# alberto-paparella/MusicRecommendation

Measured on AMD Instinct MI355X. Metric: scored (test-user,song) pairs/sec, ItemBasedModel, 1/2/4/8 MI355X + mAP@10, higher is better.
Workload: dtype int64

## Files before the change

include/mr_engine.h:

```cpp
#ifndef MR_ENGINE_H
#define MR_ENGINE_H

#include <stdint.h>
#include <stddef.h>

#ifdef __cplusplus
extern "C" {
#endif

#define MR_OK          0
#define MR_E_INVALID  -1
#define MR_E_HIP      -2
#define MR_E_OOM      -3
#define MR_E_STATE    -4
#define MR_E_IO       -5
#define MR_E_PARSE    -6
#define MR_E_RCCL     -7

#define MR_UBM 0
#define MR_IBM 1

#define MR_OUT_F32 0
#define MR_OUT_F64 1

// ... 35 lines not shown

int mr_create(const mr_options* opt, mr_ctx** out);
int mr_destroy(mr_ctx* ctx);

int mr_load(mr_ctx* ctx, const mr_dataset* d);

int mr_shard_info(const mr_ctx* ctx, int32_t* song_lo, int32_t* song_hi, int32_t* n_test_users);

int mr_launch_info(const mr_ctx* ctx, int32_t* shape, int32_t* block_songs, int32_t* n_tiles);

int mr_batch_info(const mr_ctx* ctx, int32_t* batch, int32_t* chunk, int32_t* n_chunks);

int mr_route_info(const mr_ctx* ctx, int32_t* route, int32_t* n_rows, int64_t* pool_entries);

int mr_topk_mode(const mr_ctx* ctx, int32_t* candidate_only);

int mr_cooc_stats(mr_ctx* ctx, int64_t* index_nnz, int64_t* consumed, int64_t* build_reads);

typedef struct mr_cooc_bytes_t {
  int64_t heavy_rows, light_rows;
  int64_t heavy_reads, light_reads;
  int64_t heavy_index_bytes, light_index_bytes;
  int64_t heavy_visits;
  int64_t consumed_bytes;
  int64_t group_tiles;
  int64_t n_groups;
  int64_t index_sparse_entries, index_dense_songs;
  int64_t consumed_sparse_entries, consumed_dense_songs;
} mr_cooc_bytes_t;
int mr_cooc_bytes(mr_ctx* ctx, mr_cooc_bytes_t* out);
// ... 174 lines not shown
```

musicrecommendation_amd/_lib.py:

```python
from __future__ import annotations

import ctypes
import os
from ctypes import POINTER, c_char_p, c_double, c_int, c_int32, c_int64, c_void_p

_HERE = os.path.dirname(os.path.abspath(__file__))
_VARIANT = os.environ.get("MR_ENGINE_LIB", "")
LIB_PATH = os.path.join(_HERE, f"libmr_engine_{_VARIANT}.so" if _VARIANT else "libmr_engine.so")

MR_OK = 0
MR_E_INVALID = -1
MR_E_HIP = -2
MR_E_OOM = -3
MR_E_STATE = -4
MR_E_IO = -5
MR_E_PARSE = -6
MR_E_RCCL = -7
MR_TRANSPORT_AUTO, MR_TRANSPORT_COPY, MR_TRANSPORT_RCCL = 0, 1, 2
MR_UBM = 0
MR_IBM = 1
STAGE1 = {"auto": 0, "fused": 1, "separate": 2, "wide": 4}
SHAPES = {0: "separate", 1: "fused", 3: "wide"}
MR_OUT_F32 = 0
MR_OUT_F64 = 1
# ... 88 lines not shown
    def __init__(self, code: int, where: str, msg: str):
        super().__init__(f"{where}: {_ERRNAMES.get(code, code)}: {msg}")
        self.code = code


SIGNATURES = {
    "mr_options_default": (c_int, [POINTER(MrOptions)]),
    "mr_create": (c_int, [POINTER(MrOptions), POINTER(c_void_p)]),
    "mr_destroy": (c_int, [c_void_p]),
    "mr_load": (c_int, [c_void_p, POINTER(MrDataset)]),
    "mr_shard_info": (c_int, [c_void_p, POINTER(c_int32), POINTER(c_int32), POINTER(c_int32)]),
    "mr_launch_info": (c_int, [c_void_p, POINTER(c_int32), POINTER(c_int32), POINTER(c_int32)]),
    "mr_batch_info": (c_int, [c_void_p, POINTER(c_int32), POINTER(c_int32), POINTER(c_int32)]),
    "mr_route_info": (c_int, [c_void_p, POINTER(c_int32), POINTER(c_int32), POINTER(c_int64)]),
    "mr_topk_mode": (c_int, [c_void_p, POINTER(c_int32)]),
    "mr_cooc_stats": (c_int, [c_void_p, POINTER(c_int64), POINTER(c_int64), POINTER(c_int64)]),
    "mr_cooc_bytes": (c_int, [c_void_p, POINTER(MrCoocBytes)]),
    "mr_shard_tile_songs": (c_int, [POINTER(MrOptions), c_int32, c_int32, POINTER(c_int32)]),
    "mr_shard_tile_songs_n": (c_int, [POINTER(MrOptions), c_int32, c_int32, c_int32, c_int32, POINTER(c_int32)]),
    "mr_run": (c_int, [c_void_p, c_int]),
    "mr_sync": (c_int, [c_void_p]),
    "mr_graph_capture": (c_int, [c_void_p, c_int, c_int32]),
    "mr_graph_launch": (c_int, [c_void_p]),
    "mr_device_outputs": (c_int, [c_void_p, POINTER(c_void_p), POINTER(c_void_p), POINTER(c_void_p), POINTER(c_void_p)]),
    "mr_score_dense": (c_int, [c_void_p, c_int, c_void_p]),
    "mr_topk": (c_int, [c_void_p, c_int, c_int, c_void_p, c_void_p, c_void_p]),
    "mr_copy_dense": (c_int, [c_void_p, c_void_p]),
    "mr_copy_topk": (c_int, [c_void_p, c_void_p, c_void_p, c_void_p]),
    "mr_copy_topk_device": (c_int, [c_void_p, c_void_p, c_void_p]),
    "mr_copy_topk_device_async": (c_int, [c_void_p, c_void_p, c_void_p]),
# ... 112 lines not shown
```

musicrecommendation_amd/csrc/mr_engine.hip:

```cpp
#include <hip/hip_runtime.h>

#include <algorithm>
#include <atomic>
#include <climits>
#include <cmath>
#include <cstdarg>
#include <cstdio>
#include <cstdlib>
#include <cstring>
#include <limits>
#include <mutex>
#include <string>
#include <vector>

#ifndef MR_TILE_ROWS
#define MR_TILE_ROWS 32
#endif

#include "mr_engine.h"
#include "mr_internal.h"
#include "mr_par.h"


namespace {
// ... 1 lines not shown
constexpr int kThreads = 256;
constexpr int kWaves = kThreads / 64;
constexpr int kMaxTopK = 64;
constexpr int kMaxBlockSongs = 16384;
constexpr int kLdsBytes = 160 * 1024;
constexpr int kMaxWideBlockSongs = 65536;
constexpr int kMaxLdsTrainUsers = 16384;
constexpr int kStage1Chunk = 4096;
constexpr int kMaxChunks = 2048;
constexpr int kMaxFusedTrainUsers = 4096;
constexpr long long kKeyNone = -1;
constexpr int kMaxTopkTile = 1024;
constexpr int kMaxTopkLarge = 16;
constexpr int kFusedPre = 4;
constexpr int kWideMapDefault = 1;

thread_local std::string g_err = "no error";

int fail(int code, const char* fmt, ...) {
  char buf[1024];
  va_list ap;
  va_start(ap, fmt);
  vsnprintf(buf, sizeof buf, fmt, ap);
  va_end(ap);
  g_err = buf;
  return code;
}

}

// ... 73 lines not shown
#ifdef MR_STAMPS
  if (sb && threadIdx.x == 0) sb[i] = (long long)__builtin_amdgcn_s_memrealtime();
#endif
}
__device__ __forceinline__ void stamp_rt_wave(long long* sb, int i) {
#ifdef MR_STAMPS
  if (sb && (threadIdx.x & 63) == 0) sb[i] = (long long)__builtin_amdgcn_s_memrealtime();
#endif
}
__device__ __forceinline__ void stamp_val(long long* sb, int i, long long v, bool wave = false) {
#ifdef MR_STAMPS
  if (sb && (wave ? (threadIdx.x & 63) == 0 : threadIdx.x == 0)) sb[i] = v;
#endif
}
#ifdef MR_STAMPS
#define MR_STAMP(i) stamp_at(p.stamps ? p.stamps + ((size_t)blockIdx.y * gridDim.x + blockIdx.x) * kStampSlots : nullptr, (i))
#else
#define MR_STAMP(i) do {} while (0)
#endif

__device__ __forceinline__ int wave_incl_scan(int x) {
#ifndef MR_NO_DPP
  x += __builtin_amdgcn_update_dpp(0, x, 0x111, 0xf, 0xf, false);
  x += __builtin_amdgcn_update_dpp(0, x, 0x112, 0xf, 0xf, false);
  x += __builtin_amdgcn_update_dpp(0, x, 0x114, 0xf, 0xf, false);
  x += __builtin_amdgcn_update_dpp(0, x, 0x118, 0xf, 0xf, false);
  x += __builtin_amdgcn_update_dpp(0, x, 0x142, 0xa, 0xf, false);
  x += __builtin_amdgcn_update_dpp(0, x, 0x143, 0xc, 0xf, false);
#else
  const int lane = threadIdx.x & 63;
#pragma unroll
// ... 776 lines not shown
  unsigned* counter;
  long long* top_key;
  int* top_song;
  double* top_score;
  long long* stamps;
  int topk_lists;
  int n_rows, nseg;
  const int* te_row;
  const long long* seg_off;
  const int* seg_len;
  const unsigned* pool;
  unsigned long long* mm_key;
  int mm_n;
  int cand;
  const float* rsq_c;
};

template <int MODEL, typename OutT, bool FUSED>
__global__ __launch_bounds__(kThreads) void k_score(ScoreParams p) {
  extern __shared__ __align__(16) unsigned char smem_raw[];
  const int bs = p.block_songs;
  const ScoreLds L = score_lds(bs, FUSED ? p.n_tr : 0, p.topk, p.n_tiles, FUSED ? 0 : p.n_chunks);
  unsigned long long* acc = reinterpret_cast<unsigned long long*>(smem_raw + L.acc);
  unsigned* heard = reinterpret_cast<unsigned*>(smem_raw + L.heard);
  long long* wk = reinterpret_cast<long long*>(smem_raw + L.wk);
  int* ws = reinterpret_cast<int*>(smem_raw + L.ws);
  long long* fk = reinterpret_cast<long long*>(smem_raw + L.fk);
  int* fs = reinterpret_cast<int*>(smem_raw + L.fs);
  int* flag = reinterpret_cast<int*>(smem_raw + L.flag);

  int tile = blockIdx.x;
// ... 703 lines not shown
    const int e = __builtin_ctz(sm);
    sm &= sm - 1u;
    const int i = tid + e * NT;
    double score = (double)(long long)acc[i] * inv_f;
    if (MODEL == MR_IBM) score = score / p.sqrt_c[blo + i];
    const int pos = atomicAdd(counter, 1);
    if (pos < cap) { ck[pos] = __double_as_longlong(score); cs[pos] = blo + i; }
  }
  __syncthreads();
  stamp_at(sb, 11);
  const int nc = *counter;
  if (nc > cap) return false;
  rank_survivors<NT>(nc, k, ck, cs, crank, fk, fs);
  return true;
}
constexpr int kCandE = 20;

template <int MODEL, typename OutT, int NT, int KS, bool COOC>
__global__ __launch_bounds__(NT) void k_score_wide(ScoreParams p) {
  constexpr int NW = NT / 64;
  extern __shared__ __align__(16) unsigned char smem_raw[];
  const int bs = p.block_songs;
  const WideLds<NT> L = wide_lds<NT>(bs, p.topk, p.n_chunks);
  unsigned long long* acc = reinterpret_cast<unsigned long long*>(smem_raw + L.acc);
  unsigned* heard = reinterpret_cast<unsigned*>(smem_raw + L.heard);
  int* cpre = reinterpret_cast<int*>(smem_raw + L.cpre);
  int* s_scan = reinterpret_cast<int*>(smem_raw + L.s_scan);

  const int lin = blockIdx.y * gridDim.x + blockIdx.x;
  const int slot = lin >> 3;
  int bu, tile;
  if (p.xcd_remap == 2) {
    const int per_xcd = (gridDim.x * gridDim.y) >> 3;
    const int pidx = (lin & 7) * per_xcd + slot;
    tile = pidx / gridDim.y;
    bu = pidx - tile * gridDim.y;
  } else if (p.xcd_remap == 3) {
    tile = lin / gridDim.y;
    bu = lin - tile * gridDim.y;
  } else {
    bu = (slot / p.n_tiles) * 8 + (lin & 7);
    tile = slot % p.n_tiles;
  }
  if (bu >= p.n_users) return;
  const int u = p.user0 + bu;
  const int tid = threadIdx.x, lane = tid & 63, w = tid >> 6;
  const int blo = p.song_lo + tile * bs;
  const int bhi = min(p.song_hi, blo + bs);
  const int bw = bhi - blo;
  MR_STAMP(0);

  constexpr bool kPF = COOC && MR_COOC_PF > 0;
  constexpr int PF = kPF ? MR_COOC_PF : 1;
  double scp[PF];
  if constexpr (kPF) {
#pragma unroll
    for (int e = 0; e < PF; ++e) {
      const int i = tid + e * NT;
      scp[e] = i < bw ? p.sqrt_c[blo + i] : 1.0;
    }
  }
  constexpr bool kDPF = COOC && MR_COOC_DPF;
  int pf_r = -1, pf_s = 0, pf_sl = 0;
  long long pf_off = 0;
  unsigned long long pf_q = 0ull;
// ... 280 lines not shown
      for (int r = 0; r < R; ++r) {
        const int k = k0 + r * NT;
        v[r] = -1;
        q[r] = 0ull;
        if (k < cnt) {
          while (cur + 1 < nch && cpre[cur + 1] <= k) ++cur;
          const size_t idx = (size_t)cur * p.chunk + (k - cpre[cur]);
          v[r] = nv[idx];
          q[r] = (unsigned long long)nq[idx];
        }
      }
    };
    walk_tile_lists<NT, R, kSeg, unsigned long long>(tid, cnt, load_list, p.toff + (size_t)tile * p.n_tr, p.tsongs,
                                                     [&](unsigned x, unsigned long long q) { atomicAdd(&acc[x], q); });
  }
  __syncthreads();
  MR_STAMP(2);

  long long* wk = reinterpret_cast<long long*>(smem_raw + L.wk);
  int* ws = reinterpret_cast<int*>(smem_raw + L.ws);
  long long* fk = reinterpret_cast<long long*>(smem_raw + L.fk);
  int* fs = reinterpret_cast<int*>(smem_raw + L.fs);
  const int k = KS == 10 ? 10 : p.topk;
  bool have = false;
#ifdef MR_STAMPS
  long long* sbp = p.stamps ? p.stamps + ((size_t)blockIdx.y * gridDim.x + blockIdx.x) * kStampSlots : nullptr;
#else
  long long* sbp = nullptr;
#endif
  if (p.cand) {
    have = wide_cand_topk<MODEL, NT, kCandE>(p, acc, heard, blo, bw, k, smem_raw + L.gm, wk, ws,
                                             min(256, NW * k), fk, fs, sbp, have_rv, pre_rv);
    MR_STAMP(6);
  }
  if (!have) {
  const double inv_f = ldexp(1.0, -p.frac_bits);
  OutT* out = reinterpret_cast<OutT*>(p.dense_out) + (size_t)u * p.width + (blo - p.song_lo);
  long long mk = kKeyNone;
  int ms = INT_MAX;
  OutT lmn = (OutT)INFINITY, lmx = (OutT)-INFINITY;
  auto store = [&](int i, bool h, double score) {
    const OutT o = h ? (OutT)NAN : (OutT)score;
    out[i] = o;
    if (!h) {
      lmn = o < lmn ? o : lmn;
      lmx = o > lmx ? o : lmx;
    }
  };
  constexpr int EB = MR_WIDE_EB;
// ... 1109 lines not shown
    }
    __syncthreads();
    if ((tid >> 6) == 0) wave_merge_lists(nl + off, k, mk, ms, fk, fs);
    __syncthreads();
    done += nl;
    off = 1;
  }
  const size_t o = (size_t)bu * k;
  for (int r = tid; r < k; r += kThreads) {
    p.out_keys[o + r] = fk[r];
    p.out_songs[o + r] = fs[r];
    if (p.out_scores) p.out_scores[o + r] = fk[r] >= 0 ? __longlong_as_double(fk[r]) : (double)NAN;
  }
}

__global__ __launch_bounds__(256) void k_sbound(const long long* trs_off, const int* trs_users, int n_s, int nc1,
                                                int chunk, int* sbound) {
  const size_t total = (size_t)n_s * nc1;
  for (size_t i = (size_t)blockIdx.x * 256 + threadIdx.x; i < total; i += (size_t)gridDim.x * 256) {
    const int s = (int)(i / nc1);
    const long long bound = (long long)(int)(i - (size_t)s * nc1) * chunk;
    long long a = trs_off[s], b = trs_off[s + 1];
    while (a < b) {
      const long long m = (a + b) >> 1;
      if (trs_users[m] < bound) a = m + 1; else b = m;
    }
    sbound[i] = (int)a;
  }
}

// ... 85 lines not shown
  NbrKernel nbr_kernel[2] = {nullptr, nullptr};
  DevBuf<long long> tr_off, te_off, trs_off, q_song, cand_key, top_key, nbr_q;
  DevBuf<int> te_songs, trs_users, toff, nbr_v, nbr_cnt, cand_song, top_song;
  DevBuf<unsigned short> tsongs;
  DevBuf<unsigned> tpack;
  DevBuf<int2> te_rng;
  DevBuf<long long> te_q;
  DevBuf<uint2> te_sched;
  DevBuf<long long> sched_off;
  DevBuf<int> sbound;
  DevBuf<unsigned> counter;
  DevBuf<double> sqrt_c, sqrt_tr, sqrt_te, top_score;
  DevBuf<float> rsq_c;
  std::vector<int32_t> song_count;
  bool cand_on = false;
  DevBuf<unsigned char> dense;
  DevBuf<long long> stamps;
  hipEvent_t stage_ev[2] = {nullptr, nullptr};
  static constexpr int kRing = 1024;
  std::vector<hipEvent_t> ring;
  int ring_used = 0;
  bool ring_has_stage1[kRing] = {};
  long long launches[3] = {0, 0, 0};
  double ms[3] = {0, 0, 0};
  hipEvent_t win[2] = {nullptr, nullptr};
  bool win_open = false;
  bool win_stopped = false;
  void* dense_override = nullptr;
  DevBuf<unsigned long long> mm_key;
  bool mm_on = false, mm_valid = false;
// ... 19 lines not shown
  DevBuf<int4> rdesc;
  DevBuf<long long> sr_off;
  DevBuf<unsigned> sr_songs;
  DevBuf<unsigned> urec;
  DevBuf<unsigned> lrec;
  DevBuf<uint2> llrec;

  void release_data() {
    tr_off.release(); te_off.release(); trs_off.release(); q_song.release();
    cand_key.release(); top_key.release(); nbr_q.release();
    tsongs.release(); tpack.release(); te_rng.release(); te_q.release(); te_sched.release(); sched_off.release(); te_songs.release(); trs_users.release(); toff.release(); sbound.release();
    nbr_v.release(); nbr_cnt.release(); cand_song.release(); top_song.release();
    counter.release();
    sqrt_c.release(); sqrt_tr.release(); sqrt_te.release(); top_score.release();
    rsq_c.release(); cand_on = false;
    song_count = std::vector<int32_t>();
    dense.release();
    mm_key.release(); mm_on = mm_valid = false;
    stamps.release();
    flag.release();
    row_song.release(); te_row.release(); seg_len.release(); row_base.release(); seg_off.release();
    pool.release();
    rows_order.release(); row_slots.release(); sr_off.release(); sr_songs.release(); row_nnz.release();
    urec.release(); lrec.release(); llrec.release(); rdesc.release();
    cooc = CoocPlan{};
    cooc_kernel = nullptr;
    if (graph_exec) (void)hipGraphExecDestroy(graph_exec);
    if (graph) (void)hipGraphDestroy(graph);
    graph_exec = nullptr;
    graph = nullptr;
// ... 175 lines not shown
    if constexpr (MODEL == MR_IBM) {
      if (c->cooc.route == 2 && c->cooc.cooc_nt == 512) {
        if (c->opt.topk == 10)
          c->cooc_kernel = f64 ? k_score_wide<MR_IBM, double, 512, 10, true> : k_score_wide<MR_IBM, float, 512, 10, true>;
        else
          c->cooc_kernel = f64 ? k_score_wide<MR_IBM, double, 512, kMaxTopkLarge, true>
                               : k_score_wide<MR_IBM, float, 512, kMaxTopkLarge, true>;
      } else if (c->cooc.route == 2) {
        if (c->opt.topk == 10)
          c->cooc_kernel = f64 ? k_score_wide<MR_IBM, double, kWideThreads, 10, true>
                               : k_score_wide<MR_IBM, float, kWideThreads, 10, true>;
        else
          c->cooc_kernel = f64 ? k_score_wide<MR_IBM, double, kWideThreads, kMaxTopkLarge, true>
                               : k_score_wide<MR_IBM, float, kWideThreads, kMaxTopkLarge, true>;
      }
    }
  }
  c->nbr_kernel[MODEL] = k_neighbours<MODEL>;
}

int pick_shape(const mr_options& o, int n_tr, int n_te) {
  const int k = o.topk;
  if (o.stage1 == 1) return kShapeFused;
  if (o.stage1 == 2) return kShapeSeparate;
  if (o.stage1 == 4) return kShapeWide;
  if (n_tr > kMaxFusedTrainUsers && k <= kMaxTopkLarge) return kShapeWide;
  if ((long long)n_te * n_tr >= kWideMinUserPairs && k <= kMaxTopkLarge) return kShapeWide;
  return n_tr <= kMaxFusedTrainUsers ? kShapeFused : kShapeSeparate;
}

// ... 629 lines not shown
  int rc;
  if (k > 0) {
    const int cand_users = !lp.wide() ? n_te : route == 2 ? std::max(lp.batch, std::min(n_te, 65528)) : lp.batch;
    const size_t nc = (size_t)cand_users * lp.n_tiles * k;
    if ((rc = dev_alloc(c->cand_key, nc))) return rc;
    if ((rc = dev_alloc(c->cand_song, nc))) return rc;
    const size_t nk = (size_t)n_te * k;
    if ((rc = dev_alloc(c->top_key, (size_t)topk_record_bytes(nk) / 8))) return rc;
    c->top_song.p = reinterpret_cast<int*>(c->top_key.p + nk);
    c->top_song.n = nk;
    c->top_song.own = false;
    if ((rc = dev_alloc(c->top_score, (size_t)n_te * k))) return rc;
    const size_t n_ctr = lp.wide() ? (size_t)n_te : (size_t)n_te * kCounterStride;
    if ((rc = dev_alloc(c->counter, n_ctr))) return rc;
    MR_HIP(hipMemsetAsync(c->counter.p, 0, n_ctr * sizeof(unsigned), st));
  }
  const size_t esz = c->opt.out_dtype == MR_OUT_F64 ? 8 : 4;
  if ((rc = dev_alloc(c->dense, c->opt.dense ? (size_t)n_te * lp.width * esz : 1))) return rc;
  if ((rc = dev_alloc(c->flag, 1))) return rc;
  return MR_OK;
}

int setup_kernels(mr_ctx* c, const LaunchPlan& lp, int n_tr) {
  const CoocPlan& p = c->cooc;
  const int bs = lp.block_songs, k = lp.k, n_chunks = lp.n_chunks;
  const bool fused = lp.fused(), wide = lp.wide();
  {
    const char* e = std::getenv("MR_WIDE_CAND");
    const int nt = p.route == 2 ? p.cooc_nt : kWideThreads;
    c->cand_on = wide && !c->opt.dense && k >= 1 && k <= nt / 16 && !c->opt.topk_lists && bs <= kCandE * nt &&
// ... 1 lines not shown
  }
  c->wide_lds = wide ? (size_t)wide_lds<kWideThreads>(bs, k, n_chunks).total : 0;
  pick_kernels<MR_UBM>(c);
  pick_kernels<MR_IBM>(c);
  c->score_lds = wide ? c->wide_lds
                      : (size_t)score_lds(bs, fused ? n_tr : 0, k, lp.n_tiles, fused ? 0 : n_chunks).total;
  if (c->score_lds > 160 * 1024)
    return fail(MR_E_INVALID, "scoring kernel needs %zu B of LDS (> 160 KiB): lower block_songs or topk",
                c->score_lds);
  c->nbr_lds = (size_t)align16(lp.chunk * 8) + kThreads * 16 + (kThreads + 4 + kWaves) * 4;
  for (int m = 0; m < 2; ++m) {
    MR_HIP(hipFuncSetAttribute((const void*)c->score_kernel[m], hipFuncAttributeMaxDynamicSharedMemorySize,
                               (int)c->score_lds));
    MR_HIP(hipFuncSetAttribute((const void*)c->nbr_kernel[m], hipFuncAttributeMaxDynamicSharedMemorySize,
                               (int)c->nbr_lds));
  }
  if (p.route == 2) {
    const WideLds<kWideThreads> WL = p.cooc_nt == 512 ? wide_lds<512>(bs, k, n_chunks).as_wide()
                                                      : wide_lds<kWideThreads>(bs, k, n_chunks);
    c->cooc_score_lds = (size_t)WL.total;
    c->nseg = std::min(std::min(p.cooc_nt, (WL.total - WL.wk - 8) / 40), 255);
    if (c->nseg < 16) return fail(MR_E_INVALID, "co-listening route: no LDS for row descriptors");
    c->cooc_lds = (size_t)cooc_build_lds<false>(bs);
    if (p.grp > 0)
      MR_HIP(hipFuncSetAttribute(p.group_nt == 512 ? (const void*)k_cooc_group<512> : (const void*)k_cooc_group<1024>,
                                 hipFuncAttributeMaxDynamicSharedMemorySize, cooc_group_lds(bs, p.grp)));
    for (int t = 0; t < kLightTiers; ++t)
      if (int rc2 = light_tier_call(t, nullptr, 0, nullptr, CoocParams{})) return rc2;
    MR_HIP(hipFuncSetAttribute((const void*)c->cooc_kernel, hipFuncAttributeMaxDynamicSharedMemorySize,
                               (int)c->cooc_score_lds));
    MR_HIP(hipFuncSetAttribute((const void*)k_cooc_build<MR_COOC_NT, false>, hipFuncAttributeMaxDynamicSharedMemorySize,
                               (int)c->cooc_lds));
    MR_HIP(hipFuncSetAttribute((const void*)k_cooc_build<MR_COOC_NT16, true>, hipFuncAttributeMaxDynamicSharedMemorySize,
                               cooc_build_lds<true>(bs)));
  }
  if (wide && k > 0) {
    c->merge_lds = (size_t)merge_lds_bytes(k);
    MR_HIP(hipFuncSetAttribute((const void*)k_topk_merge, hipFuncAttributeMaxDynamicSharedMemorySize,
                               (int)c->merge_lds));
  }
  return MR_OK;
}

}
// ... 174 lines not shown
  if (!c) return fail(MR_E_INVALID, "null context");
  if (!c->loaded) return fail(MR_E_STATE, "mr_route_info before mr_load");
  if (route) *route = c->cooc.route;
  if (n_rows) *n_rows = c->cooc.n_rows();
  if (pool_entries) *pool_entries = c->cooc.pool_cap;
  return MR_OK;
}

int mr_topk_mode(const mr_ctx* c, int32_t* candidate_only) {
  if (!c || !candidate_only) return fail(MR_E_INVALID, "null argument");
  if (!c->loaded) return fail(MR_E_STATE, "mr_topk_mode before mr_load");
  *candidate_only = c->cand_on ? 1 : 0;
  return MR_OK;
}

int mr_cooc_stats(mr_ctx* c, int64_t* index_nnz, int64_t* consumed, int64_t* build_reads) {
  if (!c) return fail(MR_E_INVALID, "null context");
  if (!c->loaded || c->cooc.route != 2) return fail(MR_E_STATE, "mr_cooc_stats needs a context on ibm_route 2");
  if (!c->cooc_ran) return fail(MR_E_STATE, "mr_cooc_stats before an ibm run");
  MR_HIP(hipSetDevice(c->opt.device));
  std::vector<unsigned> nnz((size_t)std::max(1, c->cooc.n_rows()), 0u);
  if (c->cooc.n_rows() > 0)
    MR_HIP(hipMemcpyAsync(nnz.data(), c->row_nnz.p, (size_t)c->cooc.n_rows() * 4, hipMemcpyDeviceToHost, c->stream));
  MR_HIP(hipStreamSynchronize(c->stream));
  int64_t tot = 0, use = 0;
  for (int r = 0; r < c->cooc.n_rows(); ++r) {
    tot += nnz[r];
    use += (int64_t)nnz[r] * c->cooc.row_users[r];
  }
  if (index_nnz) *index_nnz = tot;
// ... 102 lines not shown

}

namespace {

int flush_timing(mr_ctx* c) {
  if (c->ring_used == 0) return MR_OK;
  MR_HIP(hipEventSynchronize(c->ring[(size_t)(c->ring_used - 1) * 3 + 2]));
  for (int i = 0; i < c->ring_used; ++i) {
    hipEvent_t* e = &c->ring[(size_t)i * 3];
    float t;
    if (c->ring_has_stage1[i]) { MR_HIP(hipEventElapsedTime(&t, e[0], e[1])); c->ms[0] += t; c->launches[0]++; }
    MR_HIP(hipEventElapsedTime(&t, e[1], e[2])); c->ms[1] += t; c->launches[1]++;
  }
  c->ring_used = 0;
  return MR_OK;
}

int run_cooc(mr_ctx* c) {
  hipStream_t st = c->stream;
  const CoocPlan& p = c->cooc;
  const bool timed = c->opt.time_kernels != 0;
  const int k = c->opt.topk;
  hipEvent_t* ev = nullptr;
  if (timed) {
    if (c->ring_used == mr_ctx::kRing) {
      int rc = flush_timing(c);
      if (rc) return rc;
    }
    ev = &c->ring[(size_t)c->ring_used * 3];
// ... 59 lines not shown
      lp.rows = c->rows_order.p + lr;
      lp.rdesc = c->rdesc.p + lr;
      lp.llrec = reinterpret_cast<const unsigned*>(c->llrec.p);
      lp.lstamps = c->stamps.p ? c->stamps.p + c->lstamp_off + (size_t)(lr - p.n_heavy()) * 8 : nullptr;
      hipStream_t ls = side ? c->side[t < 2 ? 0 : 1] : st;
      if (int rc2 = light_tier_call(t, ls, p.n_light_tier[t], &lp, lp)) return rc2;
      lr += p.n_light_tier[t];
    }
    if (side)
      for (int i = 0; i < 2; ++i) {
        MR_HIP(hipEventRecord(c->side_join[i], c->side[i]));
        MR_HIP(hipStreamWaitEvent(st, c->side_join[i], 0));
      }
  }
  if (timed) MR_HIP(hipEventRecord(ev[1], st));
  const int rows = mr_internal::launch_rows(65528);
  for (int y0 = 0; y0 < c->n_te; y0 += rows) {
    const int ny = std::min(rows, c->n_te - y0);
    const int remap = wide_map_opt();
    ScoreParams sp{};
    sp.chunk = c->chunk; sp.n_chunks = c->n_chunks;
    sp.n_users = ny; sp.xcd_remap = remap;
    sp.merge_rows = merge_rows_opt();
    sp.n_tr = c->n_tr;
    sp.user0 = y0;
    sp.song_lo = c->song_lo; sp.song_hi = c->song_hi; sp.width = c->width;
    sp.block_songs = c->block_songs; sp.n_tiles = c->n_tiles;
    sp.frac_bits = c->opt.frac_bits; sp.topk = k; sp.dense = c->opt.dense;
    sp.te_off = c->te_off.p; sp.te_songs = c->te_songs.p;
    sp.sqrt_c = c->sqrt_c.p; sp.q_song = c->q_song.p;
    sp.n_rows = p.n_rows(); sp.nseg = c->nseg;
    sp.te_row = c->te_row.p; sp.seg_off = c->seg_off.p; sp.seg_len = c->seg_len.p; sp.pool = c->pool.p;
    sp.dense_out = c->dense_override ? c->dense_override : (void*)c->dense.p;
    sp.cand_key = c->cand_key.p; sp.cand_song = c->cand_song.p; sp.counter = c->counter.p;
    sp.top_key = c->top_key.p; sp.top_song = c->top_song.p; sp.top_score = c->top_score.p;
    sp.stamps = y0 == 0 ? c->stamps.p : nullptr;
    sp.topk_lists = c->opt.topk_lists;
    if (c->mm_on) { sp.mm_key = c->mm_key.p; sp.mm_n = c->n_te; }
    sp.cand = c->cand_on && !sp.mm_key; sp.rsq_c = c->rsq_c.p;
    hipLaunchKernelGGL(c->cooc_kernel, dim3(c->n_tiles, (ny + 7) / 8 * 8), dim3(p.cooc_nt), c->cooc_score_lds, st, sp);
    MR_HIP(hipGetLastError());
    if (k > 0 && c->n_tiles > 1) {
      MergeParams mp{c->n_tiles, k, k, (long long)c->n_tiles * k, (long long)k, (long long)k, c->cand_key.p,
                     c->cand_song.p, c->top_key.p + (size_t)y0 * k, c->top_song.p + (size_t)y0 * k,
                     c->top_score.p + (size_t)y0 * k};
      hipLaunchKernelGGL(k_topk_merge, dim3(ny), dim3(kThreads), c->merge_lds, st, mp);
      MR_HIP(hipGetLastError());
    }
    if (c->win_open) c->win_launches++;
  }
  if (timed) MR_HIP(hipEventRecord(ev[2], st));
  return MR_OK;
}

int ensure_nbr(mr_ctx* c) {
  if (c->shape == kShapeFused || (c->nbr_v.p && c->nbr_q.p && c->nbr_cnt.p)) return MR_OK;
// ... 1 lines not shown
  if ((rc = dev_alloc(c->nbr_v, (size_t)c->batch * c->cap))) return rc;
  if ((rc = dev_alloc(c->nbr_q, (size_t)c->batch * c->cap))) return rc;
  if ((rc = dev_alloc(c->nbr_cnt, (size_t)c->batch * c->n_chunks))) return rc;
  return MR_OK;
}

int run_model(mr_ctx* c, int model) {
  if (model == MR_IBM && c->cooc.route == 2) {
    c->cooc_ran = true;
    return run_cooc(c);
  }
  hipStream_t st = c->stream;
  const bool timed = c->opt.time_kernels != 0;
  const int k = c->opt.topk;
  const int rows1 = mr_internal::launch_rows(65535), rows = mr_internal::launch_rows(65528);
  for (int user0 = 0; user0 < c->n_te; user0 += c->batch) {
    const int nb = std::min(c->batch, c->n_te - user0);
    hipEvent_t* ev = nullptr;
    if (timed) {
      if (c->ring_used == mr_ctx::kRing) {
        int rc = flush_timing(c);
        if (rc) return rc;
      }
      ev = &c->ring[(size_t)c->ring_used * 3];
      c->ring_has_stage1[c->ring_used] = c->shape != kShapeFused;
      c->ring_used++;
      MR_HIP(hipEventRecord(ev[0], st));
    }
    if (c->shape == kShapeSeparate || c->shape == kShapeWide) {
      if (!c->nbr_v.p || !c->nbr_q.p || !c->nbr_cnt.p) {
// ... 37 lines not shown
      sp.te_rng = nullptr;
#endif
      sp.trs_off = c->trs_off.p; sp.trs_users = c->trs_users.p; sp.q_song = c->q_song.p;
      sp.sqrt_tr = c->sqrt_tr.p; sp.sqrt_te = c->sqrt_te.p;
      sp.cap = c->cap;
      sp.nbr_v = c->fused ? nullptr : c->nbr_v.p + (size_t)y0 * c->cap;
      sp.nbr_q = c->fused ? nullptr : c->nbr_q.p + (size_t)y0 * c->cap;
      sp.nbr_cnt = c->fused ? nullptr : c->nbr_cnt.p + (size_t)y0 * c->n_chunks;
      sp.dense_out = c->dense_override ? c->dense_override : (void*)c->dense.p;
      sp.cand_key = c->cand_key.p; sp.cand_song = c->cand_song.p; sp.counter = c->counter.p;
      sp.top_key = c->top_key.p; sp.top_song = c->top_song.p; sp.top_score = c->top_score.p;
      sp.stamps = c->stamps.p ? c->stamps.p + (size_t)y0 * c->n_tiles * kStampSlots : nullptr;
      sp.topk_lists = c->opt.topk_lists;
      if (c->mm_on && wide) { sp.mm_key = c->mm_key.p; sp.mm_n = c->n_te; }
      sp.cand = wide && c->cand_on && !sp.mm_key; sp.rsq_c = c->rsq_c.p;
      hipLaunchKernelGGL(c->score_kernel[model], dim3(c->n_tiles, gy), dim3(wide ? kWideThreads : kThreads),
                         c->score_lds, st, sp);
      MR_HIP(hipGetLastError());
      if (wide && k > 0 && c->n_tiles > 1) {
        MergeParams mp{c->n_tiles, k, k, (long long)c->n_tiles * k, (long long)k, (long long)k, c->cand_key.p, c->cand_song.p,
                       c->top_key.p + (size_t)(user0 + y0) * k, c->top_song.p + (size_t)(user0 + y0) * k,
                       c->top_score.p + (size_t)(user0 + y0) * k};
        hipLaunchKernelGGL(k_topk_merge, dim3(ny), dim3(kThreads), c->merge_lds, st, mp);
        MR_HIP(hipGetLastError());
      }
      if (c->win_open) c->win_launches++;
    }
    if (timed) MR_HIP(hipEventRecord(ev[2], st));
  }
  return MR_OK;
}

}
// ... 458 lines not shown
```

musicrecommendation_amd/engine.py:

```python
from __future__ import annotations

import ctypes
from typing import Optional, Tuple, Union

import numpy as np

from . import _lib
from .dataset import Dataset

MODELS = {"ubm": _lib.MR_UBM, "ibm": _lib.MR_IBM, _lib.MR_UBM: _lib.MR_UBM, _lib.MR_IBM: _lib.MR_IBM}
KERNELS = {"neighbours": 0, "score": 1}
IBM_ROUTES = {"auto": 0, "two_hop": 1, "cooc": 2}


def model_id(model: Union[str, int]) -> int:
    try:
        return MODELS[model]
    except KeyError:
        raise ValueError(f"unknown model {model!r}: use 'ubm' or 'ibm'") from None


class Engine:
    def __init__(self, dataset: Dataset, *, device: int = 0, frac_bits: int = 32, song_lo: int = 0,
                 song_hi: int = 0, block_songs: int = 0, out_dtype: str = "f32", topk: int = 10,
# ... 65 lines not shown

    def __del__(self):
        try:
            self.close()
        except Exception:
            pass

    def run(self, model: Union[str, int]) -> None:
        _lib.check(self._L.mr_run(self._h, model_id(model)), "mr_run")

    def cooc_stats(self) -> Tuple[int, int, int]:
        a, b, c = ctypes.c_int64(), ctypes.c_int64(), ctypes.c_int64()
        _lib.check(self._L.mr_cooc_stats(self._h, ctypes.byref(a), ctypes.byref(b), ctypes.byref(c)), "mr_cooc_stats")
        return a.value, b.value, c.value

    def cooc_bytes(self) -> dict:
        b = _lib.MrCoocBytes()
        _lib.check(self._L.mr_cooc_bytes(self._h, ctypes.byref(b)), "mr_cooc_bytes")
        return {name: int(getattr(b, name)) for name, _t in _lib.MrCoocBytes._fields_}

    def sync(self) -> None:
        _lib.check(self._L.mr_sync(self._h), "mr_sync")

    def graph_capture(self, model: Union[str, int], n_steps: int) -> None:
        _lib.check(self._L.mr_graph_capture(self._h, model_id(model), int(n_steps)), "mr_graph_capture")

    def graph_launch(self) -> None:
        _lib.check(self._L.mr_graph_launch(self._h), "mr_graph_launch")

    @property
# ... 298 lines not shown
```

Baseline: 16.96 billion.

## Split wide scoring into two passes using a per-user top-k threshold from early tiles

Wide scoring now runs in two launches. The first launch scores the first two song tiles per user, and a small kernel merges their candidate lists into a per-user k-th-best threshold. The second launch scores the remaining tiles and uses that threshold to keep only survivors at or above it. This is meant to cut candidate-selection work in later tiles. The cost is an extra launch, a serialization point between the passes, and a fallback to the full candidate path whenever survivors overflow the buffer.

```diff
diff --git a/include/mr_engine.h b/include/mr_engine.h
--- a/include/mr_engine.h
+++ b/include/mr_engine.h
@@ -73,6 +73,9 @@
 int mr_route_info(const mr_ctx* ctx, int32_t* route, int32_t* n_rows, int64_t* pool_entries);
 
 int mr_topk_mode(const mr_ctx* ctx, int32_t* candidate_only);
+
+int mr_topk_slice_stats(mr_ctx* ctx, int32_t* slice_tiles, int64_t* users_with_threshold,
+                        int64_t* fallback_workgroups);
 
 int mr_cooc_stats(mr_ctx* ctx, int64_t* index_nnz, int64_t* consumed, int64_t* build_reads);
 
diff --git a/musicrecommendation_amd/_lib.py b/musicrecommendation_amd/_lib.py
--- a/musicrecommendation_amd/_lib.py
+++ b/musicrecommendation_amd/_lib.py
@@ -126,6 +126,7 @@
     "mr_batch_info": (c_int, [c_void_p, POINTER(c_int32), POINTER(c_int32), POINTER(c_int32)]),
     "mr_route_info": (c_int, [c_void_p, POINTER(c_int32), POINTER(c_int32), POINTER(c_int64)]),
     "mr_topk_mode": (c_int, [c_void_p, POINTER(c_int32)]),
+    "mr_topk_slice_stats": (c_int, [c_void_p, POINTER(c_int32), POINTER(c_int64), POINTER(c_int64)]),
     "mr_cooc_stats": (c_int, [c_void_p, POINTER(c_int64), POINTER(c_int64), POINTER(c_int64)]),
     "mr_cooc_bytes": (c_int, [c_void_p, POINTER(MrCoocBytes)]),
     "mr_shard_tile_songs": (c_int, [POINTER(MrOptions), c_int32, c_int32, POINTER(c_int32)]),
diff --git a/musicrecommendation_amd/csrc/mr_engine.hip b/musicrecommendation_amd/csrc/mr_engine.hip
--- a/musicrecommendation_amd/csrc/mr_engine.hip
+++ b/musicrecommendation_amd/csrc/mr_engine.hip
@@ -39,6 +39,8 @@
 constexpr int kMaxTopkLarge = 16;
 constexpr int kFusedPre = 4;
 constexpr int kWideMapDefault = 1;
+constexpr int kWideSliceDefault = 2;
+constexpr long long kWideSliceMinWork = 65536;
 
 thread_local std::string g_err = "no error";
 
@@ -142,7 +144,7 @@
 #endif
 }
 #ifdef MR_STAMPS
-#define MR_STAMP(i) stamp_at(p.stamps ? p.stamps + ((size_t)blockIdx.y * gridDim.x + blockIdx.x) * kStampSlots : nullptr, (i))
+#define MR_STAMP(i) stamp_at(p.stamps ? p.stamps + stamp_slot(p) * kStampSlots : nullptr, (i))
 #else
 #define MR_STAMP(i) do {} while (0)
 #endif
@@ -949,7 +951,29 @@
   int mm_n;
   int cand;
   const float* rsq_c;
+  int tile0, tile_cnt;
+  const long long* slice_thr;
+  unsigned* slice_fallback;
 };
+
+#ifdef MR_STAMPS
+__device__ __forceinline__ size_t stamp_slot(const ScoreParams& p) {
+  const int lin = blockIdx.y * gridDim.x + blockIdx.x;
+  if (p.tile_cnt <= 0 || p.tile_cnt == p.n_tiles) return (size_t)lin;
+  const int gy = gridDim.y;
+  if (p.xcd_remap == 2) {
+    const int per = (gridDim.x * gy) >> 3, pidx = (lin & 7) * per + (lin >> 3);
+    const int t = pidx / gy, full = (p.tile0 + t) * gy + (pidx - t * gy), fper = (p.n_tiles * gy) >> 3;
+    return ((size_t)(full % fper) << 3) | (size_t)(full / fper);
+  }
+  if (p.xcd_remap == 3) {
+    const int t = lin / gy;
+    return (size_t)(p.tile0 + t) * gy + (lin - t * gy);
+  }
+  const int slot = lin >> 3, g = slot / p.tile_cnt, t = p.tile0 + slot % p.tile_cnt;
+  return ((size_t)(g * p.n_tiles + t) << 3) | (size_t)(lin & 7);
+}
+#endif
 
 template <int MODEL, typename OutT, bool FUSED>
 __global__ __launch_bounds__(kThreads) void k_score(ScoreParams p) {
@@ -1683,9 +1707,85 @@
   rank_survivors<NT>(nc, k, ck, cs, crank, fk, fs);
   return true;
 }
+#ifndef MR_SLICE_INLINE
+#define MR_SLICE_INLINE 0
+#endif
+template <int MODEL, int NT, int EMAX>
+__device__ __forceinline__ bool wide_cand_slice(const ScoreParams& p, const unsigned long long* acc,
+                                                const unsigned* heard, int blo, int bw, int k, long long thr_key,
+                                                unsigned char* gm, long long* ck, int* cs, int cap, long long* fk,
+                                                int* fs, long long* sb, bool have_rv,
+                                                const float (&pre_rv)[MR_CAND_EB]) {
+  constexpr int NG = NT / 16;
+  const int tid = threadIdx.x;
+  int* counter = reinterpret_cast<int*>(reinterpret_cast<long long*>(gm) + NG + 1) + NG + 1;
+  int* crank = counter + 1 + NG;
+  const float thr = __double2float_rz(__longlong_as_double(thr_key) * ldexp(1.0, p.frac_bits)) * (1.f - 0x1p-17f);
+  const double inv_f = ldexp(1.0, -p.frac_bits);
+  unsigned sm = 0u;
+  auto drain = [&]() {
+    while (sm) {
+      const int i = tid + __builtin_ctz(sm) * NT;
+      sm &= sm - 1u;
+      double score = (double)(long long)acc[i] * inv_f;
+      if (MODEL == MR_IBM) score = score / p.sqrt_c[blo + i];
+      const int pos = atomicAdd(counter, 1);
+      if (pos < cap) { ck[pos] = __double_as_longlong(score); cs[pos] = blo + i; }
+    }
+  };
+  if (MR_SLICE_INLINE) {
+    stamp_at(sb, 3);
+    stamp_at(sb, 9);
+    stamp_at(sb, 10);
+  }
+  constexpr int EB = MR_CAND_EB;
+#pragma unroll
+  for (int e0 = 0; e0 < EMAX; e0 += EB) {
+    unsigned long long av[EB];
+    float rv[EB];
+#pragma unroll
+    for (int j = 0; j < EB; ++j) {
+      const int i = tid + (e0 + j) * NT;
+      av[j] = 0ull;
+      rv[j] = 0.f;
+      if (e0 + j < EMAX && i < bw) {
+        av[j] = acc[i];
+        rv[j] = MODEL != MR_IBM ? 1.f : (e0 == 0 && have_rv) ? pre_rv[j] : p.rsq_c[blo + i];
+      }
+    }
+#pragma unroll
+    for (int j = 0; j < EB; ++j) {
+      const int i = tid + (e0 + j) * NT;
+      float a = -1.f;
+      if (e0 + j < EMAX && i < bw && !((heard[i >> 5] >> (i & 31)) & 1u)) {
+        const float hi = (float)(unsigned)(av[j] >> 32), lo = (float)(unsigned)av[j];
+        a = __fmaf_rn(hi, 4294967296.f, lo) * rv[j];
+      }
+      sm |= a >= thr ? 1u << (e0 + j) : 0u;
+    }
+    if (MR_SLICE_INLINE) drain();
+  }
+  if (!MR_SLICE_INLINE) {
+    stamp_at(sb, 3);
+    stamp_at(sb, 9);
+    stamp_at(sb, 10);
+    drain();
+  }
+  __syncthreads();
+  stamp_at(sb, 11);
+  const int nc = *counter;
+  if (nc > cap) {
+    if (tid == 0) atomicAdd(p.slice_fallback, 1u);
+    __syncthreads();
+    return false;
+  }
+  rank_survivors<NT>(nc, k, ck, cs, crank, fk, fs);
+  return true;
+}
+
 constexpr int kCandE = 20;
 
-template <int MODEL, typename OutT, int NT, int KS, bool COOC>
+template <int MODEL, typename OutT, int NT, int KS, bool COOC, bool SLICE = false>
 __global__ __launch_bounds__(NT) void k_score_wide(ScoreParams p) {
   constexpr int NW = NT / 64;
   extern __shared__ __align__(16) unsigned char smem_raw[];
@@ -1708,9 +1808,10 @@
     tile = lin / gridDim.y;
     bu = lin - tile * gridDim.y;
   } else {
-    bu = (slot / p.n_tiles) * 8 + (lin & 7);
-    tile = slot % p.n_tiles;
-  }
+    bu = (slot / p.tile_cnt) * 8 + (lin & 7);
+    tile = slot % p.tile_cnt;
+  }
+  tile += p.tile0;
   if (bu >= p.n_users) return;
   const int u = p.user0 + bu;
   const int tid = threadIdx.x, lane = tid & 63, w = tid >> 6;
@@ -1718,6 +1819,8 @@
   const int bhi = min(p.song_hi, blo + bs);
   const int bw = bhi - blo;
   MR_STAMP(0);
+  long long thr_key = -1;
+  if constexpr (SLICE) thr_key = p.slice_thr[u];
 
   constexpr bool kPF = COOC && MR_COOC_PF > 0;
   constexpr int PF = kPF ? MR_COOC_PF : 1;
@@ -2028,6 +2131,13 @@
     walk_tile_lists<NT, R, kSeg, unsigned long long>(tid, cnt, load_list, p.toff + (size_t)tile * p.n_tr, p.tsongs,
                                                      [&](unsigned x, unsigned long long q) { atomicAdd(&acc[x], q); });
   }
+  if constexpr (SLICE) {
+    if (p.cand && thr_key > 0) {
+      int* counter = reinterpret_cast<int*>(reinterpret_cast<long long*>(smem_raw + L.gm) + NT / 16 + 1) + NT / 16 + 1;
+      if (tid == 0) *counter = 0;
+      if (tid < 256) counter[1 + NT / 16 + tid] = 0;
+    }
+  }
   __syncthreads();
   MR_STAMP(2);
 
@@ -2038,15 +2148,20 @@
   const int k = KS == 10 ? 10 : p.topk;
   bool have = false;
 #ifdef MR_STAMPS
-  long long* sbp = p.stamps ? p.stamps + ((size_t)blockIdx.y * gridDim.x + blockIdx.x) * kStampSlots : nullptr;
+  long long* sbp = p.stamps ? p.stamps + stamp_slot(p) * kStampSlots : nullptr;
 #else
   long long* sbp = nullptr;
 #endif
-  if (p.cand) {
+  if constexpr (SLICE) {
+    if (p.cand && thr_key > 0)
+      have = wide_cand_slice<MODEL, NT, kCandE>(p, acc, heard, blo, bw, k, thr_key, smem_raw + L.gm, wk, ws,
+                                                min(256, NW * k), fk, fs, sbp, have_rv, pre_rv);
+  }
+  if (p.cand && !have) {
     have = wide_cand_topk<MODEL, NT, kCandE>(p, acc, heard, blo, bw, k, smem_raw + L.gm, wk, ws,
                                              min(256, NW * k), fk, fs, sbp, have_rv, pre_rv);
-    MR_STAMP(6);
-  }
+  }
+  if (p.cand) MR_STAMP(6);
   if (!have) {
   const double inv_f = ldexp(1.0, -p.frac_bits);
   OutT* out = reinterpret_cast<OutT*>(p.dense_out) + (size_t)u * p.width + (blo - p.song_lo);
@@ -3186,6 +3301,24 @@
   }
 }
 
+__global__ __launch_bounds__(256) void k_slice_thr(const long long* cand_key, int n_users, int n_tiles, int n_a, int k,
+                                                   long long* thr, unsigned* fallback_reset) {
+  const int bu = blockIdx.x * 256 + threadIdx.x;
+  if (bu == 0 && fallback_reset) *fallback_reset = 0u;
+  if (bu >= n_users) return;
+  const long long* a = cand_key + (size_t)bu * n_tiles * k;
+  const long long* b = a + k;
+  int ha = 0, hb = 0;
+  long long v = kKeyNone;
+  for (int r = 0; r < k; ++r) {
+    const long long x = ha < k ? a[ha] : kKeyNone, y = n_a > 1 && hb < k ? b[hb] : kKeyNone;
+    v = x >= y ? x : y;
+    ha += x >= y ? 1 : 0;
+    hb += x >= y ? 0 : 1;
+  }
+  thr[bu] = v > 0 ? v : -1;
+}
+
 __global__ __launch_bounds__(256) void k_sbound(const long long* trs_off, const int* trs_users, int n_s, int nc1,
                                                 int chunk, int* sbound) {
   const size_t total = (size_t)n_s * nc1;
@@ -3301,6 +3434,11 @@
   DevBuf<float> rsq_c;
   std::vector<int32_t> song_count;
   bool cand_on = false;
+  ScoreKernel slice_kernel[2] = {nullptr, nullptr}, cooc_slice_kernel = nullptr;
+  DevBuf<long long> slice_thr;
+  DevBuf<unsigned> slice_fb;
+  int slice_tiles = 0;
+  bool slice_fresh = false;
   DevBuf<unsigned char> dense;
   DevBuf<long long> stamps;
   hipEvent_t stage_ev[2] = {nullptr, nullptr};
@@ -3350,6 +3488,7 @@
     counter.release();
     sqrt_c.release(); sqrt_tr.release(); sqrt_te.release(); top_score.release();
     rsq_c.release(); cand_on = false;
+    slice_thr.release(); slice_fb.release(); slice_tiles = 0;
     song_count = std::vector<int32_t>();
     dense.release();
     mm_key.release(); mm_on = mm_valid = false;
@@ -3555,6 +3694,16 @@
           c->cooc_kernel = f64 ? k_score_wide<MR_IBM, double, kWideThreads, kMaxTopkLarge, true>
                                : k_score_wide<MR_IBM, float, kWideThreads, kMaxTopkLarge, true>;
       }
+    }
+    c->slice_kernel[MODEL] = c->opt.topk == 10 ? k_score_wide<MODEL, float, kWideThreads, 10, false, true>
+                                               : k_score_wide<MODEL, float, kWideThreads, kMaxTopkLarge, false, true>;
+    if constexpr (MODEL == MR_IBM) {
+      if (c->cooc.route == 2 && c->cooc.cooc_nt == 512)
+        c->cooc_slice_kernel = c->opt.topk == 10 ? k_score_wide<MR_IBM, float, 512, 10, true, true>
+                                                 : k_score_wide<MR_IBM, float, 512, kMaxTopkLarge, true, true>;
+      else if (c->cooc.route == 2)
+        c->cooc_slice_kernel = c->opt.topk == 10 ? k_score_wide<MR_IBM, float, kWideThreads, 10, true, true>
+                                                 : k_score_wide<MR_IBM, float, kWideThreads, kMaxTopkLarge, true, true>;
     }
   }
   c->nbr_kernel[MODEL] = k_neighbours<MODEL>;
@@ -4214,6 +4363,12 @@
     const size_t n_ctr = lp.wide() ? (size_t)n_te : (size_t)n_te * kCounterStride;
     if ((rc = dev_alloc(c->counter, n_ctr))) return rc;
     MR_HIP(hipMemsetAsync(c->counter.p, 0, n_ctr * sizeof(unsigned), st));
+    if (lp.wide()) {
+      if ((rc = dev_alloc(c->slice_thr, (size_t)n_te))) return rc;
+      if ((rc = dev_alloc(c->slice_fb, 1))) return rc;
+      MR_HIP(hipMemsetAsync(c->slice_thr.p, 0xff, (size_t)std::max(1, n_te) * sizeof(long long), st));
+      MR_HIP(hipMemsetAsync(c->slice_fb.p, 0, sizeof(unsigned), st));
+    }
   }
   const size_t esz = c->opt.out_dtype == MR_OUT_F64 ? 8 : 4;
   if ((rc = dev_alloc(c->dense, c->opt.dense ? (size_t)n_te * lp.width * esz : 1))) return rc;
@@ -4245,6 +4400,9 @@
                                (int)c->score_lds));
     MR_HIP(hipFuncSetAttribute((const void*)c->nbr_kernel[m], hipFuncAttributeMaxDynamicSharedMemorySize,
                                (int)c->nbr_lds));
+    if (wide)
+      MR_HIP(hipFuncSetAttribute((const void*)c->slice_kernel[m], hipFuncAttributeMaxDynamicSharedMemorySize,
+                                 (int)c->score_lds));
   }
   if (p.route == 2) {
     const WideLds<kWideThreads> WL = p.cooc_nt == 512 ? wide_lds<512>(bs, k, n_chunks).as_wide()
@@ -4259,6 +4417,8 @@
     for (int t = 0; t < kLightTiers; ++t)
       if (int rc2 = light_tier_call(t, nullptr, 0, nullptr, CoocParams{})) return rc2;
     MR_HIP(hipFuncSetAttribute((const void*)c->cooc_kernel, hipFuncAttributeMaxDynamicSharedMemorySize,
+                               (int)c->cooc_score_lds));
+    MR_HIP(hipFuncSetAttribute((const void*)c->cooc_slice_kernel, hipFuncAttributeMaxDynamicSharedMemorySize,
                                (int)c->cooc_score_lds));
     MR_HIP(hipFuncSetAttribute((const void*)k_cooc_build<MR_COOC_NT, false>, hipFuncAttributeMaxDynamicSharedMemorySize,
                                (int)c->cooc_lds));
@@ -4463,6 +4623,29 @@
   return MR_OK;
 }
 
+int mr_topk_slice_stats(mr_ctx* c, int32_t* slice_tiles, int64_t* users_with_threshold,
+                        int64_t* fallback_workgroups) {
+  if (!c) return fail(MR_E_INVALID, "null context");
+  if (!c->loaded) return fail(MR_E_STATE, "mr_topk_slice_stats before mr_load");
+  MR_HIP(hipSetDevice(c->opt.device));
+  MR_HIP(hipStreamSynchronize(c->stream));
+  if (slice_tiles) *slice_tiles = c->slice_tiles;
+  if (users_with_threshold) *users_with_threshold = 0;
+  if (fallback_workgroups) *fallback_workgroups = 0;
+  if (c->slice_tiles <= 0) return MR_OK;
+  if (users_with_threshold) {
+    std::vector<long long> thr((size_t)c->n_te);
+    MR_HIP(hipMemcpy(thr.data(), c->slice_thr.p, thr.size() * sizeof(long long), hipMemcpyDeviceToHost));
+    for (long long v : thr) *users_with_threshold += v > 0 ? 1 : 0;
+  }
+  if (fallback_workgroups) {
+    unsigned fb = 0;
+    MR_HIP(hipMemcpy(&fb, c->slice_fb.p, sizeof(unsigned), hipMemcpyDeviceToHost));
+    *fallback_workgroups = fb;
+  }
+  return MR_OK;
+}
+
 int mr_cooc_stats(mr_ctx* c, int64_t* index_nnz, int64_t* consumed, int64_t* build_reads) {
   if (!c) return fail(MR_E_INVALID, "null context");
   if (!c->loaded || c->cooc.route != 2) return fail(MR_E_STATE, "mr_cooc_stats needs a context on ibm_route 2");
@@ -4595,6 +4778,45 @@
     MR_HIP(hipEventElapsedTime(&t, e[1], e[2])); c->ms[1] += t; c->launches[1]++;
   }
   c->ring_used = 0;
+  return MR_OK;
+}
+
+int wide_slice_opt(int n_tiles, int n_te) {
+  const char* e = std::getenv("MR_WIDE_SLICE");
+  const int v = e && e[0] ? std::atoi(e) : -1;
+  if (v >= 0 && v <= 2) return v;
+  return (long long)(n_tiles - kWideSliceDefault) * n_te >= kWideSliceMinWork ? kWideSliceDefault : 0;
+}
+
+void slice_begin_run(mr_ctx* c) {
+  c->slice_tiles = 0;
+  c->slice_fresh = true;
+}
+
+int launch_score_wide(mr_ctx* c, ScoreKernel full, ScoreKernel after, ScoreParams sp, int gy, int nt, size_t lds) {
+  hipStream_t st = c->stream;
+  const int n_a = wide_slice_opt(sp.n_tiles, c->n_te);
+  sp.tile0 = 0;
+  sp.tile_cnt = sp.n_tiles;
+  if (n_a <= 0 || !sp.cand || sp.n_tiles <= n_a || !after) {
+    hipLaunchKernelGGL(full, dim3(sp.n_tiles, gy), dim3(nt), lds, st, sp);
+    MR_HIP(hipGetLastError());
+    return MR_OK;
+  }
+  sp.tile_cnt = n_a;
+  hipLaunchKernelGGL(full, dim3(n_a, gy), dim3(nt), lds, st, sp);
+  MR_HIP(hipGetLastError());
+  hipLaunchKernelGGL(k_slice_thr, dim3((sp.n_users + 255) / 256), dim3(256), 0, st, sp.cand_key, sp.n_users, sp.n_tiles,
+                     n_a, sp.topk, c->slice_thr.p + sp.user0, c->slice_fresh ? c->slice_fb.p : nullptr);
+  MR_HIP(hipGetLastError());
+  c->slice_fresh = false;
+  sp.tile0 = n_a;
+  sp.tile_cnt = sp.n_tiles - n_a;
+  sp.slice_thr = c->slice_thr.p;
+  sp.slice_fallback = c->slice_fb.p;
+  hipLaunchKernelGGL(after, dim3(sp.tile_cnt, gy), dim3(nt), lds, st, sp);
+  MR_HIP(hipGetLastError());
+  c->slice_tiles = n_a;
   return MR_OK;
 }
 
@@ -4684,6 +4906,7 @@
       }
   }
   if (timed) MR_HIP(hipEventRecord(ev[1], st));
+  slice_begin_run(c);
   const int rows = mr_internal::launch_rows(65528);
   for (int y0 = 0; y0 < c->n_te; y0 += rows) {
     const int ny = std::min(rows, c->n_te - y0);
@@ -4708,8 +4931,9 @@
     sp.topk_lists = c->opt.topk_lists;
     if (c->mm_on) { sp.mm_key = c->mm_key.p; sp.mm_n = c->n_te; }
     sp.cand = c->cand_on && !sp.mm_key; sp.rsq_c = c->rsq_c.p;
-    hipLaunchKernelGGL(c->cooc_kernel, dim3(c->n_tiles, (ny + 7) / 8 * 8), dim3(p.cooc_nt), c->cooc_score_lds, st, sp);
-    MR_HIP(hipGetLastError());
+    if (int rc = launch_score_wide(c, c->cooc_kernel, c->cooc_slice_kernel, sp, (ny + 7) / 8 * 8, p.cooc_nt,
+                                   c->cooc_score_lds))
+      return rc;
     if (k > 0 && c->n_tiles > 1) {
       MergeParams mp{c->n_tiles, k, k, (long long)c->n_tiles * k, (long long)k, (long long)k, c->cand_key.p,
                      c->cand_song.p, c->top_key.p + (size_t)y0 * k, c->top_song.p + (size_t)y0 * k,
@@ -4741,6 +4965,7 @@
   const bool timed = c->opt.time_kernels != 0;
   const int k = c->opt.topk;
   const int rows1 = mr_internal::launch_rows(65535), rows = mr_internal::launch_rows(65528);
+  if (c->shape == kShapeWide) slice_begin_run(c);
   for (int user0 = 0; user0 < c->n_te; user0 += c->batch) {
     const int nb = std::min(c->batch, c->n_te - user0);
     hipEvent_t* ev = nullptr;
@@ -4808,9 +5033,14 @@
       sp.topk_lists = c->opt.topk_lists;
       if (c->mm_on && wide) { sp.mm_key = c->mm_key.p; sp.mm_n = c->n_te; }
       sp.cand = wide && c->cand_on && !sp.mm_key; sp.rsq_c = c->rsq_c.p;
-      hipLaunchKernelGGL(c->score_kernel[model], dim3(c->n_tiles, gy), dim3(wide ? kWideThreads : kThreads),
-                         c->score_lds, st, sp);
-      MR_HIP(hipGetLastError());
+      if (wide) {
+        if (int rc = launch_score_wide(c, c->score_kernel[model], c->slice_kernel[model], sp, gy, kWideThreads,
+                                       c->score_lds))
+          return rc;
+      } else {
+        hipLaunchKernelGGL(c->score_kernel[model], dim3(c->n_tiles, gy), dim3(kThreads), c->score_lds, st, sp);
+        MR_HIP(hipGetLastError());
+      }
       if (wide && k > 0 && c->n_tiles > 1) {
         MergeParams mp{c->n_tiles, k, k, (long long)c->n_tiles * k, (long long)k, (long long)k, c->cand_key.p, c->cand_song.p,
                        c->top_key.p + (size_t)(user0 + y0) * k, c->top_song.p + (size_t)(user0 + y0) * k,
diff --git a/musicrecommendation_amd/engine.py b/musicrecommendation_amd/engine.py
--- a/musicrecommendation_amd/engine.py
+++ b/musicrecommendation_amd/engine.py
@@ -103,6 +103,12 @@
         _lib.check(self._L.mr_cooc_stats(self._h, ctypes.byref(a), ctypes.byref(b), ctypes.byref(c)), "mr_cooc_stats")
         return a.value, b.value, c.value
 
+    def topk_slice_stats(self) -> Tuple[int, int, int]:
+        a, b, c = ctypes.c_int32(), ctypes.c_int64(), ctypes.c_int64()
+        _lib.check(self._L.mr_topk_slice_stats(self._h, ctypes.byref(a), ctypes.byref(b), ctypes.byref(c)),
+                   "mr_topk_slice_stats")
+        return a.value, b.value, c.value
+
     def cooc_bytes(self) -> dict:
         b = _lib.MrCoocBytes()
         _lib.check(self._L.mr_cooc_bytes(self._h, ctypes.byref(b)), "mr_cooc_bytes")
```

Result: no change. 16.94 billion, median of 2 (-0.1%).
